# jacobkrantz/VLN-CE

Hardware: AMD Instinct MI355X
Metric: policy-steps/sec (fwd+bwd) (higher is better)
Workload: dtype f32

## Files before the change

vln-ce_amd/_lib.py:

```python
import ctypes as C
import os
import threading

import torch

_HERE = os.path.dirname(os.path.abspath(__file__))
LIB_PATH = os.environ.get("VLNCE_HIP_LIB") or os.path.join(_HERE, "libvlnce_hip.so")

_P = C.c_void_p
_I = C.c_int
_F = C.c_float
_L = C.c_long


def _buffer_format(explicit, *bufs):
    tags = {getattr(b, "_vlnce_fmt", None) for b in bufs if b is not None} - {None}
    if explicit:
        tags.add(int(explicit))
    if len(tags) > 1:
        raise RuntimeError(f"weight buffers / w_format disagree on the plane format: {sorted(tags)}")
    return tags.pop() if tags else 1


class ConvDesc(C.Structure):
# ... 102 lines not shown
    "vlnce_adaptive_avgpool_bwd": (_I, [_P, _P, _I, _I, _I, _I, _I, _I, _P]),
    "vlnce_rnn_seq_supported": (_I, [_I, _I]),
    "vlnce_rnn_seq_fwd": (_I, [_I, _I, _P, _P, _P, _P, _P, _P, _P, _P, _I, _I, _I, _P]),
    "vlnce_rnn_seq_bwd": (_I, [_I, _I, _P, _P, _P, _P, _P, _P, _P, _P, _P, _I, _I, _I, _P]),
    "vlnce_option_count": (_I, []),
    "vlnce_option_index": (_I, [C.c_char_p]),
    "vlnce_linear_rows_supported": (_I, [_I, _I, _I]),
    "vlnce_linear_rows_fwd": (_I, [_P, _I, _P, _I, _P, _I, _P, _I, _I, _I, _I, _P]),
    "vlnce_linear_rows_bwd": (_I, [_P, _I, _P, _I, _P, _I, _P, _I, _I, _P, _P, _P, _I, _I, _I, _P]),
    "vlnce_rnn_seq_fwd2": (_I, [_I, _I, _P, _P, _P, _P, _P, _P, _L, _L, _P, _P, _P, _I, _I, _I, _P]),
    "vlnce_rnn_seq_bwd2": (_I, [_I, _I, _P, _P, _P, _P, _P, _P, _L, _L, _P, _P, _P, _P, _I, _I, _I, _P]),
    "vlnce_rnn_seq_wgrad": (_I, [_I, _I, _I, _P, _P, _P, _P, _I, _I, _P, _P, _P, _P, _P, _P, _I, _I, _I, _P]),
    "vlnce_group_norm_small": (_I, [_P, _I, _I, _I, _I, _P, _P, _F, _P, _I, _P, _P]),
    "vlnce_gru_rollout_supported": (_I, [_I, _I]),
    "vlnce_gru_rollout_workspace_bytes": (C.c_long, [_I, _I]),
    "vlnce_gru_rollout_fwd": (_I, [_P, _P, _P, _P, _P, _P, _P, _P, _P, _P, _I, _I, _I, _P]),
    "vlnce_gru_rollout_bwd": (_I, [_P, _P, _P, _P, _P, _P, _P, _P, _P, _P, _P, _I, _I, _I, _P]),
    "vlnce_rnn_step_supported": (_I, [_I, _I, _I]),
    "vlnce_rnn_step_fwd": (_I, [_I, _P, _P, _P, _P, _P, _P, _P, _P, _P, _P, _I, _I, _P]),
    "vlnce_rnn_step_bwd": (_I, [_I, _P, _P, _P, _P, _P, _P, _P, _P, _P, _P, _P, _P, _P, _I, _I, _P]),
    "vlnce_select_rows": (_I, [_P, _P, _P, _P, _I, _I, _P]),
    "vlnce_act_bwd": (_I, [_P, _P, _P, _L, _I, _P]),
}


def exported_symbols():
    return sorted(_SIGNATURES)


def load_cdll(path=LIB_PATH):
    if not os.path.exists(path):
        raise RuntimeError(
            f"{path} not found: build it with `python __graft_entry__.py` (hipcc, gfx950). "
            "The VLN-CE policy path has no CPU fallback."
        )
    dll = C.CDLL(path)
    for name, (res, args) in _SIGNATURES.items():
        fn = getattr(dll, name)
        fn.restype = res
        fn.argtypes = args
    return dll


class _CallState(threading.local):
    dev = None
    restore = None


_CALL = _CallState()


def _ptr(t):
    if t is None:
        return None
    if not t.is_cuda:
        raise RuntimeError("libvlnce_hip: tensor is not on a GPU (no CPU fallback)")
    idx = t.device.index
    if _CALL.dev is None:
        _CALL.dev = idx
    elif _CALL.dev != idx:
        first, _CALL.dev = _CALL.dev, None
        raise RuntimeError(f"libvlnce_hip: tensors of one call live on cuda:{first} and "
                           f"cuda:{idx}")
    return t.data_ptr()


def _stream():
    dev, _CALL.dev = _CALL.dev, None
    if dev is None:
        return torch.cuda.current_stream().cuda_stream
    cur = torch.cuda.current_device()
    if dev != cur:
        _CALL.restore = cur
        torch.cuda.set_device(dev)
    return torch.cuda.current_stream(dev).cuda_stream


def _leave_device():
    if _CALL.restore is not None:
        cur, _CALL.restore = _CALL.restore, None
        torch.cuda.set_device(cur)


class HipLib:

    name = "hip"

    ABI = 143

    def __init__(self, path=LIB_PATH):
        self.dll = load_cdll(path)
        have = int(self.dll.vlnce_version())
        if have != self.ABI:
            raise RuntimeError(f"{path} has ABI {have}, this package binds ABI {self.ABI}: "
                               "rebuild it (python __graft_entry__.py)")

        self._conv_math = None
        self._tls = threading.local()
        self._options_from_env()

    OPTION_NAMES = ("conv_math", "p3", "p3_tile", "s3", "u3", "u3_waves", "x3_tile", "igemm_tile",
                    "igemm_nobuf", "igemm_no_splitk", "wgrad_tile", "rollout_one_xcd", "m3")

    def _options_from_env(self):
        for name in self.OPTION_NAMES:
            v = os.environ.get("VLNCE_" + name.upper())
            if v is None:
                continue
            if name == "conv_math":
                v = {"f32": 0, "0": 0, "bf16": 1, "1": 1, "f16": 2, "2": 2}.get(v.strip().lower(), v)
            elif name in ("igemm_nobuf", "igemm_no_splitk"):
                v = 0 if v in ("", "0") else 1
            try:
                v = int(v)
            except ValueError:
                import warnings
                warnings.warn(f"VLNCE_{name.upper()}={v!r} is not an integer: ignored "
                              f"(the option keeps its default)")
                continue
            self.set_option(name, v)

    def set_option(self, name, value):
        self._check(self.dll.vlnce_set_option(name.encode(), int(value)), "vlnce_set_option")
        if name == "conv_math":
            self._conv_math = int(value)

    def plane_format(self, options=None):
        v = None
        if options:
            v = options.get("conv_math")
        if v is None:
            sc = getattr(self._tls, "scoped", None)
            if sc:
                v = sc.get("conv_math")
        if v is None or v < 0:
            v = self._conv_math
            if v is None:
                v = self._conv_math = self.get_option("conv_math")
        return 2 if v == 2 else 1

    def get_option(self, name):
        v = _I(0)
        self._check(self.dll.vlnce_get_option(name.encode(), C.byref(v)), "vlnce_get_option")
        return v.value

    def option_default(self, name):
        v = _I(0)
        self._check(self.dll.vlnce_option_default(name.encode(), C.byref(v)), "vlnce_option_default")
        return v.value

    PER_LAUNCH = ("conv_math", "p3", "p3_tile", "s3", "u3", "u3_waves", "x3_tile", "m3")

    def _launch_options(self, overrides):
        if not overrides:
            return None
        arr = (C.c_int * int(self.dll.vlnce_option_count()))(*([-1] * int(self.dll.vlnce_option_count())))
        for name, v in overrides.items():
            i = int(self.dll.vlnce_option_index(name.encode()))
            if i < 0:
                raise RuntimeError(f"unknown dispatch option {name!r}")
            arr[i] = int(v)
        return arr

    def options(self, **kw):
        lib = self
        unknown = [k for k in kw if k not in self.OPTION_NAMES]
        if unknown:
            raise RuntimeError(f"unknown dispatch option(s) {unknown}")

        class _Scope:
            def __enter__(self_inner):
                self_inner.prev = getattr(lib._tls, "scoped", None)
                scoped = dict(self_inner.prev or {})
                scoped.update({k: v for k, v in kw.items() if k in lib.PER_LAUNCH})
                lib._tls.scoped = scoped or None
                self_inner.old = {k: lib.get_option(k) for k in kw if k not in lib.PER_LAUNCH}
                for k in self_inner.old:
                    lib.set_option(k, kw[k])
                return lib

            def __exit__(self_inner, *exc):
                lib._tls.scoped = self_inner.prev
                for k, v in self_inner.old.items():
                    lib.set_option(k, v)
                return False
# ... 338 lines not shown

    def gn_bwd_workspace_floats(self, Nimg, HW, Cc, groups):
        return int(self.dll.vlnce_gn_bwd_workspace_floats(Nimg, HW, Cc, groups))

    def gn_bwd(self, dy, y, x, mean, rstd, gamma, Nimg, HW, Cc, groups, relu, dx, dres, dgamma,
               dbeta, workspace, pow2=None):
        self._check(self.dll.vlnce_gn_bwd(_ptr(dy), _ptr(y), _ptr(x), _ptr(mean), _ptr(rstd),
                                          _ptr(gamma), Nimg, HW, Cc, groups, int(relu), _ptr(dx),
                                          _ptr(dres), _ptr(dgamma), _ptr(dbeta), _ptr(workspace),
                                          _ptr(pow2), pow2.size(1) if pow2 is not None else 0,
                                          _stream()), "vlnce_gn_bwd")

    def maxpool3x3s2_argmax(self, x, y, argmax, N, H, W, Cc, Ho, Wo):
        self._check(self.dll.vlnce_maxpool3x3s2_argmax(_ptr(x), _ptr(y), _ptr(argmax), N, H, W, Cc,
                                                       Ho, Wo, _stream()),
                    "vlnce_maxpool3x3s2_argmax")

    def maxpool3x3s2_bwd(self, dy, argmax, dx, N, H, W, Cc, Ho, Wo):
        self._check(self.dll.vlnce_maxpool3x3s2_bwd(_ptr(dy), _ptr(argmax), _ptr(dx), N, H, W, Cc,
                                                    Ho, Wo, _stream()), "vlnce_maxpool3x3s2_bwd")

    def adaptive_avgpool_bwd(self, dy, dx, N, H, W, Cc, OH, OW):
        self._check(self.dll.vlnce_adaptive_avgpool_bwd(_ptr(dy), _ptr(dx), N, H, W, Cc, OH, OW,
                                                        _stream()), "vlnce_adaptive_avgpool_bwd")

    @staticmethod
    def _parr(ts, n):
        if ts is None:
            return None
        arr = (C.c_void_p * 2)()
        for i in range(n):
            arr[i] = _ptr(ts[i])
        return arr

    def rnn_seq_supported(self, kind, H):
        return bool(self.dll.vlnce_rnn_seq_supported(kind, H))

    def rnn_seq_fwd(self, kind, dirs, gi, w_hh, b_hh, lengths, out, h_final, gates_save, aux_save,
                    B, Lm, H):
        pa = self._parr
        self._check(self.dll.vlnce_rnn_seq_fwd(
            kind, dirs, pa(gi, dirs), pa(w_hh, dirs), pa(b_hh, dirs), _ptr(lengths), pa(out, dirs),
            pa(h_final, dirs), pa(gates_save, dirs), pa(aux_save, dirs), B, Lm, H, _stream()),
            "vlnce_rnn_seq_fwd")

    def rnn_seq_bwd(self, kind, dirs, w_hh_t, lengths, out, gates_save, aux_save, dout, dh_final,
                    dgi, dgh, B, Lm, H):
        pa = self._parr
        self._check(self.dll.vlnce_rnn_seq_bwd(
            kind, dirs, pa(w_hh_t, dirs), _ptr(lengths), pa(out, dirs), pa(gates_save, dirs),
            pa(aux_save, dirs), pa(dout, dirs), pa(dh_final, dirs), pa(dgi, dirs), pa(dgh, dirs),
            B, Lm, H, _stream()), "vlnce_rnn_seq_bwd")

    def linear_rows_supported(self, M, N, K):
        return bool(self.dll.vlnce_linear_rows_supported(M, N, K))

    def linear_rows_fwd(self, x, ldx, w, ldw, bias, act, y, ldy, M, N, K):
        self._check(self.dll.vlnce_linear_rows_fwd(_ptr(x), ldx, _ptr(w), ldw, _ptr(bias), act, _ptr(y),
                                                   ldy, M, N, K, _stream()), "vlnce_linear_rows_fwd")

    def linear_rows_bwd(self, x, ldx, w, ldw, dy, lddy, y, ldy, act, dx, dw, db, M, N, K):
        self._check(self.dll.vlnce_linear_rows_bwd(_ptr(x), ldx, _ptr(w), ldw, _ptr(dy), lddy, _ptr(y),
                                                   ldy, act, _ptr(dx), _ptr(dw), _ptr(db), M, N, K,
                                                   _stream()), "vlnce_linear_rows_bwd")

    def rnn_seq_fwd2(self, kind, dirs, gi, w_hh, b_hh, lengths, out_tm, seq, seq_st, seq_sb, h_final,
                     gates_save, aux_save, B, Lm, H):
        pa = self._parr
        self._check(self.dll.vlnce_rnn_seq_fwd2(
            kind, dirs, pa(gi, dirs), pa(w_hh, dirs), pa(b_hh, dirs), _ptr(lengths), pa(out_tm, dirs),
            _ptr(seq), seq_st, seq_sb, pa(h_final, dirs), pa(gates_save, dirs), pa(aux_save, dirs),
            B, Lm, H, _stream()), "vlnce_rnn_seq_fwd2")

    def rnn_seq_bwd2(self, kind, dirs, w_hh, lengths, out_tm, gates_save, aux_save, dseq, dseq_st,
                     dseq_sb, dout_ws, dh_final, dgi, dgh, B, Lm, H):
        pa = self._parr
        self._check(self.dll.vlnce_rnn_seq_bwd2(
            kind, dirs, pa(w_hh, dirs), _ptr(lengths), pa(out_tm, dirs), pa(gates_save, dirs),
            pa(aux_save, dirs), _ptr(dseq), dseq_st, dseq_sb, _ptr(dout_ws), pa(dh_final, dirs),
            pa(dgi, dirs), pa(dgh, dirs), B, Lm, H, _stream()), "vlnce_rnn_seq_bwd2")

    def rnn_seq_wgrad(self, kind, dirs, dgi, dgh, out_tm, x_tm, ldx, E, w_ih, dw_ih, dw_hh, db_ih,
                      db_hh, dx_tm, B, Lm, H, first_dir=0):
        pa = self._parr
        self._check(self.dll.vlnce_rnn_seq_wgrad(
            kind, dirs, first_dir, pa(dgi, dirs), pa(dgh, dirs), pa(out_tm, dirs), _ptr(x_tm), ldx, E,
            pa(w_ih, dirs), pa(dw_ih, dirs), pa(dw_hh, dirs), pa(db_ih, dirs), pa(db_hh, dirs),
            _ptr(dx_tm), B, Lm, H, _stream()), "vlnce_rnn_seq_wgrad")

    def group_norm_small(self, x, N, HW, Cc, groups, gamma, beta, eps, residual, act, y):
        self._check(self.dll.vlnce_group_norm_small(
            _ptr(x), N, HW, Cc, groups, _ptr(gamma), _ptr(beta), eps, _ptr(residual), act, _ptr(y),
            _stream()), "vlnce_group_norm_small")

    def gru_rollout_supported(self, N, H):
        if os.environ.get("VLNCE_GRU_ROLLOUT", "1") == "0":
            return False
        return bool(self.dll.vlnce_gru_rollout_supported(N, H))

    def gru_rollout_workspace_bytes(self, N, H):
        return int(self.dll.vlnce_gru_rollout_workspace_bytes(N, H))

    def gru_rollout_fwd(self, gi, h0, mask, w_hh, b_hh, hp, out, gates, aux, workspace, T, N, H):
        self._check(self.dll.vlnce_gru_rollout_fwd(
            _ptr(gi), _ptr(h0), _ptr(mask), _ptr(w_hh), _ptr(b_hh), _ptr(hp), _ptr(out),
            _ptr(gates), _ptr(aux), _ptr(workspace), T, N, H, _stream()), "vlnce_gru_rollout_fwd")

    def gru_rollout_bwd(self, dout, dh_final, gates, aux, hp, mask, w_hh_t, dgi, dgh, dh0,
                        workspace, T, N, H):
        self._check(self.dll.vlnce_gru_rollout_bwd(
            _ptr(dout), _ptr(dh_final), _ptr(gates), _ptr(aux), _ptr(hp), _ptr(mask),
            _ptr(w_hh_t), _ptr(dgi), _ptr(dgh), _ptr(dh0), _ptr(workspace), T, N, H, _stream()),
            "vlnce_gru_rollout_bwd")

    def rnn_step_supported(self, N, H, lstm):
        if os.environ.get("VLNCE_RNN_STEP_FUSED", "1") == "0":
            return False
        return bool(self.dll.vlnce_rnn_step_supported(N, H, int(lstm)))

    def rnn_step_fwd(self, lstm, gi, h_prev, c_prev, mask, w_hh, b_hh, hp_out, h_out, aux_out,
                     gates_out, N, H):
        self._check(self.dll.vlnce_rnn_step_fwd(
            int(lstm), _ptr(gi), _ptr(h_prev), _ptr(c_prev), _ptr(mask), _ptr(w_hh), _ptr(b_hh),
            _ptr(hp_out), _ptr(h_out), _ptr(aux_out), _ptr(gates_out), N, H, _stream()),
            "vlnce_rnn_step_fwd")

    def rnn_step_bwd(self, lstm, dout, carry, dc, gates, aux, hp, c_prev, mask, w_hh_t, dgi, dgh,
                     acc0, dc_prev, N, H):
        self._check(self.dll.vlnce_rnn_step_bwd(
            int(lstm), _ptr(dout), _ptr(carry), _ptr(dc), _ptr(gates), _ptr(aux), _ptr(hp),
            _ptr(c_prev), _ptr(mask), _ptr(w_hh_t), _ptr(dgi), _ptr(dgh), _ptr(acc0),
            _ptr(dc_prev), N, H, _stream()), "vlnce_rnn_step_bwd")

    def select_rows(self, mask, a, b, out, B, H):
        self._check(self.dll.vlnce_select_rows(_ptr(mask), _ptr(a), _ptr(b), _ptr(out), B, H,
                                               _stream()), "vlnce_select_rows")

    def embedding_bwd(self, tokens, grad_rows, grad_weight, padding_idx):
        self._check(self.dll.vlnce_embedding_bwd(_ptr(tokens), _ptr(grad_rows), _ptr(grad_weight),
                                                 tokens.numel(), grad_weight.size(1),
                                                 -1 if padding_idx is None else int(padding_idx),
                                                 grad_weight.size(0), _stream()),
                    "vlnce_embedding_bwd")

    def act_bwd(self, dy, y, dz, n, act):
        self._check(self.dll.vlnce_act_bwd(_ptr(dy), _ptr(y), _ptr(dz), n, act, _stream()),
                    "vlnce_act_bwd")


_LIB = None


def get_lib():
    global _LIB
    if _LIB is None:
        _LIB = HipLib()
    return _LIB
```

vln-ce_amd/csrc/api.cpp:

```cpp
#include <stdarg.h>
#include <stdio.h>
#include <string.h>

#include <atomic>

#include "common_opts.h"

static thread_local char g_err[512] = "";

void vlnce_set_error(const char* fmt, ...) {
  va_list ap;
  va_start(ap, fmt);
  vsnprintf(g_err, sizeof(g_err), fmt, ap);
  va_end(ap);
}

extern "C" const char* vlnce_last_error(void) { return g_err; }
extern "C" int vlnce_version(void) { return 143; }

namespace {
struct OptDef {
  const char* name;
  int def;
};
const OptDef kOpts[VLNCE_OPT_COUNT] = {
    {"conv_math", 2},   {"p3", 2},          {"p3_tile", 0},         {"s3", 1},
    {"u3", 1},          {"u3_waves", 8},    {"x3_tile", 0},         {"igemm_tile", 0},
    {"igemm_nobuf", 0}, {"igemm_no_splitk", 0}, {"wgrad_tile", 64}, {"rollout_one_xcd", 0},
    {"m3", 1},
};
std::atomic<int> g_opt[VLNCE_OPT_COUNT] = {
    {2}, {2}, {0}, {1}, {1}, {8}, {0}, {0}, {0}, {0}, {64}, {0}, {1},
};
int opt_index(const char* name) {
  if (name)
    for (int i = 0; i < VLNCE_OPT_COUNT; ++i)
      if (strcmp(name, kOpts[i].name) == 0) return i;
  return -1;
}
}

namespace {
thread_local const int* t_call_opts = nullptr;
}
VlnceOptScope::VlnceOptScope(const int* per_call) : prev(t_call_opts) { t_call_opts = per_call; }
VlnceOptScope::~VlnceOptScope() { t_call_opts = prev; }

int vlnce_opt(int id) {
  if (t_call_opts && t_call_opts[id] >= 0) return t_call_opts[id];
  return g_opt[id].load(std::memory_order_relaxed);
}

extern "C" int vlnce_option_count(void) { return VLNCE_OPT_COUNT; }

extern "C" int vlnce_option_index(const char* name) { return opt_index(name); }

extern "C" int vlnce_set_option(const char* name, int value) {
  const int i = opt_index(name);
  if (i < 0) {
    vlnce_set_error("vlnce_set_option: unknown option '%s'", name ? name : "(null)");
    return 1;
  }
  g_opt[i].store(value, std::memory_order_relaxed);
  return 0;
}

extern "C" int vlnce_get_option(const char* name, int* value) {
  const int i = opt_index(name);
  if (i < 0 || !value) {
    vlnce_set_error("vlnce_get_option: unknown option '%s'", name ? name : "(null)");
    return 1;
  }
  *value = g_opt[i].load(std::memory_order_relaxed);
  return 0;
}

extern "C" int vlnce_option_default(const char* name, int* value) {
  const int i = opt_index(name);
  if (i < 0 || !value) {
    vlnce_set_error("vlnce_option_default: unknown option '%s'", name ? name : "(null)");
    return 1;
  }
  *value = kOpts[i].def;
  return 0;
}
```

vln-ce_amd/csrc/common_opts.h:

```cpp
#pragma once
#include "../../include/vlnce_hip.h"

void vlnce_set_error(const char* fmt, ...);

enum {
  VLNCE_OPT_CONV_MATH,
  VLNCE_OPT_P3,
  VLNCE_OPT_P3_TILE,
  VLNCE_OPT_S3,
  VLNCE_OPT_U3,
  VLNCE_OPT_U3_WAVES,
  VLNCE_OPT_X3_TILE,
  VLNCE_OPT_IGEMM_TILE,
  VLNCE_OPT_IGEMM_NOBUF,
  VLNCE_OPT_IGEMM_NO_SPLITK,
  VLNCE_OPT_WGRAD_TILE,
  VLNCE_OPT_ROLLOUT_ONE_XCD,
  VLNCE_OPT_M3,
  VLNCE_OPT_COUNT
};
int vlnce_opt(int id);

struct VlnceOptScope {
  explicit VlnceOptScope(const int* per_call);
  ~VlnceOptScope();
  const int* prev;
};
```

vln-ce_amd/csrc/rnn_seq.hip:

```cpp
#include "common.h"

namespace {

struct RnnSeqParams {
  const float* gi[2];
  const float* w_hh[2];
  const float* b_hh[2];
  float* out[2];
  float* h_final[2];
  float* gates[2];
  float* aux[2];
  const float* dout[2];
  const float* dh_final[2];
  float* dgi[2];
  float* dgh[2];
  const int* lengths;
  int B, L;
  float* seq[2];
  long seq_st, seq_sb;
  int self_zero;
  int w_plain;
};

__global__ __launch_bounds__(256) void dseq_to_time_major_kernel(const float* __restrict__ dseq, long st,
// ... 448 lines not shown
            const float dz = dht * (hp - ng);
            const float dnp = dn * (1.f - ng * ng);
            dpre[0] = dnp * hn * rg * (1.f - rg);
            dpre[1] = dz * zg * (1.f - zg);
            dpre[2] = dnp;
            dgh_n = dnp * rg;
            keep_z[nt][r] = dht * zg;
          }
          float* dgi = p.dgi[d] + base * GH;
#pragma unroll
          for (int gt = 0; gt < G; ++gt) dgi[gt * H + u] = dpre[gt];
          if (KIND == 1) {
            float* dgh = p.dgh[d] + base * GH;
            dgh[u] = dpre[0];
            dgh[H + u] = dpre[1];
            dgh[2 * H + u] = dgh_n;
          }
        }
#pragma unroll
        for (int gt = 0; gt < G; ++gt) {
          unsigned short dw[3];
          split_scalar((KIND == 1 && gt == 2) ? dgh_n : dpre[gt], dw);
#pragma unroll
          for (int q = 0; q < 3; ++q) dg_pl[q][row_i][gt * H + u] = dw[q];
        }
      }
    }
#ifdef RNN_SEQ_DBG_TIME
    const long long d_t1 = clock64();
#endif
    __syncthreads();
#ifdef RNN_SEQ_DBG_TIME
    const long long d_t2 = clock64();
#endif
    f32x4 acc[NTW];
#pragma unroll
    for (int nt = 0; nt < NTW; ++nt) acc[nt] = f32x4{0.f, 0.f, 0.f, 0.f};
#pragma unroll
    for (int ks = 0; ks < KS; ++ks) {
      bf16x8 a[3];
#pragma unroll
      for (int q = 0; q < 3; ++q)
        a[q] = *reinterpret_cast<const bf16x8*>(&dg_pl[q][l15][32 * ks + 8 * quad]);
      Planes3 wl;
      const bool from_lds = KL > 0 && ks >= KS - KL;
      if (from_lds) {
#pragma unroll
        for (int q = 0; q < 3; ++q) wl.p[q] = w_lds[KL > 0 ? ks - (KS - KL) : 0][q][tid];
      }
#pragma unroll
      for (int q = 0; q < 6; ++q)
#pragma unroll
        for (int nt = 0; nt < NTW; ++nt) {
          const bf16x8 wb = (from_lds && nt == 0) ? wl.p[X3_PB[q]] : wt[nt][ks].p[X3_PB[q]];
          acc[nt] = __builtin_amdgcn_mfma_f32_16x16x32_bf16(a[X3_PA[q]], wb, acc[nt], 0, 0, 0);
        }
    }
#pragma unroll
    for (int r = 0; r < 4; ++r) {
      const bool active = s < len[r];
      if (active)
#pragma unroll
        for (int nt = 0; nt < NTW; ++nt) dh[nt][r] = acc[nt][r] + keep_z[nt][r];
    }
#ifdef RNN_SEQ_DBG_TIME
    const long long d_t3 = clock64();
#endif
    __syncthreads();
#ifdef RNN_SEQ_DBG_TIME
    const long long d_t4 = clock64();
    d_a += d_t1 - d_t0;
    d_b1 += d_t2 - d_t1;
    d_m += d_t3 - d_t2;
    d_b2 += d_t4 - d_t3;
#endif
  }
#ifdef RNN_SEQ_DBG_TIME
  if (blockIdx.x == 0 && blockIdx.y == 0 && (tid == 0 || tid == 64 * (NW - 1)))
    printf("rnn_seq_bwd wave %d: %d steps; per step: gates+LDS write %lld, barrier %lld, reads+MFMA %lld, "
           "barrier %lld cycles\n", wave, Lt, d_a / Lt, d_b1 / Lt, d_m / Lt, d_b2 / Lt);
#endif
}

template <int KIND>
int launch_fwd(const RnnSeqParams& p, int H, int dirs, hipStream_t s) {
  dim3 grid(ceil_div(p.B, 16), dirs);
  if (H == 64)
    hipLaunchKernelGGL((rnn_seq_fwd_kernel<KIND, 64, 4>), grid, dim3(256), 0, s, p);
  else if (H == 128)
    hipLaunchKernelGGL((rnn_seq_fwd_kernel<KIND, 128, 8>), grid, dim3(512), 0, s, p);
  else
    return 1;
  return 0;
}
template <int KIND>
int launch_bwd(const RnnSeqParams& p, int H, int dirs, hipStream_t s) {
  dim3 grid(ceil_div(p.B, 16), dirs);
  if (H == 64)
    hipLaunchKernelGGL((rnn_seq_bwd_kernel<KIND, 64, 4>), grid, dim3(256), 0, s, p);
  else if (H == 128)
    hipLaunchKernelGGL((rnn_seq_bwd_kernel<KIND, 128, 8>), grid, dim3(512), 0, s, p);
  else
    return 1;
  return 0;
}

}

extern "C" int vlnce_rnn_seq_supported(int kind, int H) {
  return (kind == 0 || kind == 1) && (H == 64 || H == 128);
}

extern "C" int vlnce_rnn_seq_fwd(int kind, int dirs, const float* const* gi,
                                 const float* const* w_hh, const float* const* b_hh,
                                 const int* lengths, float* const* out, float* const* h_final,
                                 float* const* gates_save, float* const* aux_save, int B, int L,
                                 int H, vlnce_stream_t stream) {
  VLNCE_CHECK_ARG(gi && w_hh && b_hh && lengths && out && h_final, "rnn_seq_fwd: null argument");
  VLNCE_CHECK_ARG(dirs == 1 || dirs == 2, "rnn_seq_fwd: dirs must be 1 or 2");
  VLNCE_CHECK_ARG(vlnce_rnn_seq_supported(kind, H), "rnn_seq_fwd: unsupported kind/H (%d,%d)", kind, H);
  VLNCE_CHECK_ARG(B > 0 && L > 0, "rnn_seq_fwd: bad shape");
  RnnSeqParams p{};
  for (int d = 0; d < dirs; ++d) {
    p.gi[d] = gi[d];
    p.w_hh[d] = w_hh[d];
    p.b_hh[d] = b_hh[d];
    p.out[d] = out[d];
    p.h_final[d] = h_final[d];
    p.gates[d] = gates_save ? gates_save[d] : nullptr;
    p.aux[d] = aux_save ? aux_save[d] : nullptr;
    VLNCE_CHECK_ARG((p.gates[d] == nullptr) == (p.aux[d] == nullptr),
                    "rnn_seq_fwd: gates_save and aux_save come together");
  }
  p.lengths = lengths;
  p.B = B;
  p.L = L;
  hipStream_t s = reinterpret_cast<hipStream_t>(stream);
  const int rc = kind == 0 ? launch_fwd<0>(p, H, dirs, s) : launch_fwd<1>(p, H, dirs, s);
  VLNCE_CHECK_ARG(rc == 0, "rnn_seq_fwd: no kernel for H=%d", H);
  VLNCE_CHECK_LAUNCH("rnn_seq_fwd");
  return 0;
}

extern "C" int vlnce_rnn_seq_bwd(int kind, int dirs, const float* const* w_hh_t,
                                 const int* lengths, const float* const* out,
                                 const float* const* gates_save, const float* const* aux_save,
                                 const float* const* dout, const float* const* dh_final,
                                 float* const* dgi, float* const* dgh, int B, int L, int H,
                                 vlnce_stream_t stream) {
  VLNCE_CHECK_ARG(w_hh_t && lengths && out && gates_save && aux_save && dgi,
                  "rnn_seq_bwd: null argument");
  VLNCE_CHECK_ARG(dirs == 1 || dirs == 2, "rnn_seq_bwd: dirs must be 1 or 2");
  VLNCE_CHECK_ARG(vlnce_rnn_seq_supported(kind, H), "rnn_seq_bwd: unsupported kind/H (%d,%d)", kind, H);
  VLNCE_CHECK_ARG(kind == 0 || dgh, "rnn_seq_bwd: GRU needs dgh");
  RnnSeqParams p{};
  for (int d = 0; d < dirs; ++d) {
    p.w_hh[d] = w_hh_t[d];
    p.out[d] = const_cast<float*>(out[d]);
    p.gates[d] = const_cast<float*>(gates_save[d]);
    p.aux[d] = const_cast<float*>(aux_save[d]);
    p.dout[d] = dout ? dout[d] : nullptr;
    p.dh_final[d] = dh_final ? dh_final[d] : nullptr;
    p.dgi[d] = dgi[d];
    p.dgh[d] = dgh ? dgh[d] : nullptr;
  }
  p.lengths = lengths;
// ... 22 lines not shown
  for (int d = 0; d < dirs; ++d) {
    p.gi[d] = gi[d];
    p.w_hh[d] = w_hh[d];
    p.b_hh[d] = b_hh[d];
    p.out[d] = out_tm[d];
    p.seq[d] = seq ? seq + (long)d * H : nullptr;
    p.h_final[d] = h_final[d];
    p.gates[d] = gates_save ? gates_save[d] : nullptr;
    p.aux[d] = aux_save ? aux_save[d] : nullptr;
    VLNCE_CHECK_ARG((p.gates[d] == nullptr) == (p.aux[d] == nullptr),
                    "rnn_seq_fwd2: gates_save and aux_save come together");
  }
  p.seq_st = seq_st;
  p.seq_sb = seq_sb;
  p.self_zero = 1;
  p.lengths = lengths;
  p.B = B;
  p.L = L;
  hipStream_t s = reinterpret_cast<hipStream_t>(stream);
  const int rc = kind == 0 ? launch_fwd<0>(p, H, dirs, s) : launch_fwd<1>(p, H, dirs, s);
  VLNCE_CHECK_ARG(rc == 0, "rnn_seq_fwd2: no kernel for H=%d", H);
  VLNCE_CHECK_LAUNCH("rnn_seq_fwd2");
  return 0;
}

extern "C" int vlnce_rnn_seq_bwd2(int kind, int dirs, const float* const* w_hh, const int* lengths,
                                  const float* const* out_tm, const float* const* gates_save,
                                  const float* const* aux_save, const float* dseq, long dseq_st,
                                  long dseq_sb, float* dout_ws, const float* const* dh_final,
                                  float* const* dgi, float* const* dgh, int B, int L, int H,
                                  vlnce_stream_t stream) {
  VLNCE_CHECK_ARG(w_hh && lengths && out_tm && gates_save && aux_save && dgi,
                  "rnn_seq_bwd2: null argument");
  VLNCE_CHECK_ARG(dirs == 1 || dirs == 2, "rnn_seq_bwd2: dirs must be 1 or 2");
  VLNCE_CHECK_ARG(vlnce_rnn_seq_supported(kind, H), "rnn_seq_bwd2: unsupported kind/H (%d,%d)", kind, H);
  VLNCE_CHECK_ARG(kind == 0 || dgh, "rnn_seq_bwd2: GRU needs dgh");
  VLNCE_CHECK_ARG(!dseq || (dseq_st > 0 && dseq_sb > 0), "rnn_seq_bwd2: dseq needs its strides");
  VLNCE_CHECK_ARG(!dseq || dout_ws, "rnn_seq_bwd2: dseq needs the dirs*L*B*H workspace");
  hipStream_t s = reinterpret_cast<hipStream_t>(stream);
  if (dseq) {
    const long n4 = (long)dirs * L * B * (H / 4);
    const int grid = (int)((n4 + 255) / 256 > 2048 ? 2048 : (n4 + 255) / 256);
    hipLaunchKernelGGL(dseq_to_time_major_kernel, dim3(grid), dim3(256), 0, s, dseq, dseq_st, dseq_sb,
                       dout_ws, dirs, L, B, H);
    VLNCE_CHECK_LAUNCH("rnn_seq_bwd2 (output gradient to time-major)");
  }
  RnnSeqParams p{};
  for (int d = 0; d < dirs; ++d) {
    p.w_hh[d] = w_hh[d];
    p.out[d] = const_cast<float*>(out_tm[d]);
    p.gates[d] = const_cast<float*>(gates_save[d]);
    p.aux[d] = const_cast<float*>(aux_save[d]);
    p.dout[d] = dseq ? dout_ws + (long)d * L * B * H : nullptr;
    p.dh_final[d] = dh_final ? dh_final[d] : nullptr;
    p.dgi[d] = dgi[d];
    p.dgh[d] = dgh ? dgh[d] : nullptr;
  }
  p.self_zero = 1;
  p.w_plain = 1;
  p.lengths = lengths;
  p.B = B;
  p.L = L;
  const int rc = kind == 0 ? launch_bwd<0>(p, H, dirs, s) : launch_bwd<1>(p, H, dirs, s);
  VLNCE_CHECK_ARG(rc == 0, "rnn_seq_bwd2: no kernel for H=%d", H);
  VLNCE_CHECK_LAUNCH("rnn_seq_bwd2");
  return 0;
}

extern "C" int vlnce_rnn_seq_wgrad(int kind, int dirs, int first_dir, const float* const* dgi,
                                   const float* const* dgh, const float* const* out_tm,
                                   const float* x_tm, int ldx, int E, const float* const* w_ih,
                                   float* const* dw_ih, float* const* dw_hh, float* const* db_ih,
                                   float* const* db_hh, float* dx_tm, int B, int L, int H,
                                   vlnce_stream_t stream) {
  VLNCE_CHECK_ARG(dgi && out_tm && x_tm && dw_ih && dw_hh && db_ih && db_hh,
                  "rnn_seq_wgrad: null argument");
  VLNCE_CHECK_ARG(dirs == 1 || dirs == 2, "rnn_seq_wgrad: dirs must be 1 or 2");
  VLNCE_CHECK_ARG((first_dir == 0 || first_dir == 1) && first_dir + dirs <= 2,
                  "rnn_seq_wgrad: first_dir + dirs must stay within the two directions");
  VLNCE_CHECK_ARG(kind == 0 || dgh, "rnn_seq_wgrad: GRU needs dgh");
  VLNCE_CHECK_ARG(!dx_tm || w_ih, "rnn_seq_wgrad: dx_tm needs w_ih");
  const int GH = (kind == 0 ? 4 : 3) * H;
  const long rows = (long)L * B;
  VLNCE_CHECK_ARG(B > 0 && L > 0 && E > 0 && ldx >= E && rows < 0x7fffffffL, "rnn_seq_wgrad: bad shape");
  hipStream_t s = reinterpret_cast<hipStream_t>(stream);
  for (int d = 0; d < dirs; ++d) {
    const float* dGh = kind == 1 ? dgh[d] : dgi[d];
    if (L > 1) {
      const bool reverse = first_dir + d == 1;
      const float* dG_s = reverse ? dGh : dGh + (long)B * GH;
      const float* h_s = reverse ? out_tm[d] + (long)B * H : out_tm[d];
      int rc = vlnce_gemm(dG_s, GH, 1, h_s, H, 1, dw_hh[d], H, GH, H, (int)((long)(L - 1) * B), nullptr, stream);
      if (rc != 0) return rc;
    } else {
      vlnce_zero(dw_hh[d], GH, H, H, s);
    }
    int rc = vlnce_colsum(dGh, GH, (int)rows, GH, db_hh[d], 0, stream);
    if (rc != 0) return rc;
    rc = vlnce_gemm(dgi[d], GH, 1, x_tm, ldx, 1, dw_ih[d], E, GH, E, (int)rows, nullptr, stream);
    if (rc != 0) return rc;
    if (db_ih[d] != db_hh[d]) {
      rc = vlnce_colsum(dgi[d], GH, (int)rows, GH, db_ih[d], 0, stream);
      if (rc != 0) return rc;
    }
    if (dx_tm) {
      vlnce_epilogue e{};
      e.accumulate = d > 0;
      rc = vlnce_gemm(dgi[d], GH, 0, w_ih[d], E, 1, dx_tm, E, (int)rows, E, GH, &e, stream);
      if (rc != 0) return rc;
    }
  }
  return 0;
}
```

vln-ce_amd/ops.py:

```python
import os

import torch
import torch.nn.functional as F
from torch.autograd import Function

from . import _lib

ACT_NONE, ACT_RELU, ACT_SIGMOID, ACT_TANH = 0, 1, 2, 3


def L():
    return _lib.get_lib()


def _f32c(t):
    if t.dtype != torch.float32:
        t = t.float()
    return t if t.is_contiguous() else t.contiguous()


def _rows2d(t):
    if t.dim() != 2 or t.stride(1) != 1 or (t.size(0) > 1 and t.stride(0) < t.size(1)):
        t = t.reshape(-1, t.size(-1)).contiguous()
    ld = t.stride(0) if t.size(0) > 1 else t.size(1)
# ... 940 lines not shown
            torch.mul(acc, mf[t], out=carry)
        dw = torch.empty_like(w_hh)
        lib.gemm(dgh.view(T * N, GH), GH, 1, hp.view(T * N, H), H, 1, dw, H, GH, H, T * N)
        db = torch.empty((GH,), device=dev, dtype=torch.float32)
        lib.colsum(dgh.view(T * N, GH), GH, T * N, GH, db, 0)
        dc0 = dc if lstm else None
        return None, dgi.view(T * N, GH), carry, dc0, None, dw, db


class RNNLayerFn(Function):

    @staticmethod
    def forward(ctx, kind, save, lengths, dirs, B, Lm, x_tm, *params):
        x_tm, ldx = _rows2d(_f32c(x_tm) if x_tm.dtype != torch.float32 else x_tm)
        E = x_tm.size(1)
        w_ih = [_f32c(params[4 * d]) for d in range(dirs)]
        b_ih = [params[4 * d + 1] for d in range(dirs)]
        w_hh = [_f32c(params[4 * d + 2]) for d in range(dirs)]
        b_hh = [_f32c(params[4 * d + 3]) for d in range(dirs)]
        GH, H = w_hh[0].shape
        dev = x_tm.device
        lib = L()
        rows = Lm * B
        gis = []
        for d in range(dirs):
            gi = torch.empty((rows, GH), device=dev, dtype=torch.float32)
            if not _planes_gemm(x_tm, ldx, w_ih[d], gi, b_ih[d]):
                lib.gemm(x_tm, ldx, 0, w_ih[d], E, 0, gi, GH, rows, GH, E, shift=b_ih[d])
            gis.append(gi.view(Lm, B, GH))

        def new(*shape):
            return torch.empty(shape, device=dev, dtype=torch.float32)

        out_tm = [new(Lm, B, H) for _ in range(dirs)]
        seq = new(B, Lm, dirs * H)
        hfin = [new(B, H) for _ in range(dirs)]
        gates = aux = None
        if save:
            gates = [new(Lm, B, GH) for _ in range(dirs)]
            aux = [new(Lm, B, H) for _ in range(dirs)]
        lib.rnn_seq_fwd2(kind, dirs, gis, w_hh, b_hh, lengths, out_tm, seq, dirs * H, Lm * dirs * H,
                         hfin, gates, aux, B, Lm, H)
        ctx.cfg = (kind, dirs, Lm, B, H, GH, E, ldx)
        ctx.set_materialize_grads(False)
        if save:
            ctx.save_for_backward(lengths, x_tm, *w_ih, *w_hh, *out_tm, *gates, *aux)
        return (seq, *hfin)

    @staticmethod
    def backward(ctx, dseq, *dhf):
        kind, dirs, Lm, B, H, GH, E, ldx = ctx.cfg
        sv = ctx.saved_tensors
        lengths, x_tm = sv[0], sv[1]
        w_ih, w_hh = sv[2:2 + dirs], sv[2 + dirs:2 + 2 * dirs]
        out_tm = sv[2 + 2 * dirs:2 + 3 * dirs]
        gates = sv[2 + 3 * dirs:2 + 4 * dirs]
        aux = sv[2 + 4 * dirs:2 + 5 * dirs]
        dev = x_tm.device
        st = sb = 0
        if dseq is not None:
            if (dseq.dtype != torch.float32 or dseq.stride(2) != 1 or dseq.stride(0) <= 0
                    or dseq.stride(1) <= 0):
                dseq = _f32c(dseq)
            sb, st = dseq.stride(0), dseq.stride(1)
        dhf = [(_f32c(g) if g is not None else None) for g in dhf[:dirs]]

        def new(*shape):
            return torch.empty(shape, device=dev, dtype=torch.float32)

        dgi = [new(Lm, B, GH) for _ in range(dirs)]
        dgh = [new(Lm, B, GH) for _ in range(dirs)] if kind == 1 else None
        lib = L()
        ws = new(dirs, Lm, B, H) if dseq is not None else None
        lib.rnn_seq_bwd2(kind, dirs, list(w_hh), lengths, list(out_tm), list(gates), list(aux), dseq,
                         st, sb, ws, dhf, dgi, dgh, B, Lm, H)
        dw_ih = [new(GH, E) for _ in range(dirs)]
        dw_hh = [new(GH, H) for _ in range(dirs)]
        db_ih = [new(GH) for _ in range(dirs)]
        db_hh = [new(GH) for _ in range(dirs)]
        need_dx = ctx.needs_input_grad[6]
        dx = new(Lm * B, E) if need_dx else None
        from .streams import BranchStreams

        if (dirs == 2 and Lm * B >= 2048 and BranchStreams.enabled(dev)
                and os.environ.get("VLNCE_RNN_WGRAD_STREAMS", "1") != "0"):
            cur = torch.cuda.current_stream(dev)
            side = BranchStreams()._stream(1, dev)
            if side is cur:
                side = BranchStreams()._stream(2, dev)
            dx1 = new(Lm * B, E) if need_dx else None
            fork = torch.cuda.Event()
            fork.record(cur)
            side.wait_event(fork)
            with torch.cuda.stream(side):
                lib.rnn_seq_wgrad(kind, 1, dgi[1:], dgh[1:] if dgh else None, list(out_tm[1:]), x_tm, ldx, E,
                                  list(w_ih[1:]), dw_ih[1:], dw_hh[1:], db_ih[1:], db_hh[1:], dx1, B, Lm,
                                  H, first_dir=1)
                done = torch.cuda.Event()
                done.record(side)
            lib.rnn_seq_wgrad(kind, 1, dgi[:1], dgh[:1] if dgh else None, list(out_tm[:1]), x_tm, ldx, E,
                              list(w_ih[:1]), dw_ih[:1], dw_hh[:1], db_ih[:1], db_hh[:1], dx, B, Lm, H)
            cur.wait_event(done)
            if need_dx:
                dx.add_(dx1)
        else:
            lib.rnn_seq_wgrad(kind, dirs, dgi, dgh, list(out_tm), x_tm, ldx, E, list(w_ih), dw_ih, dw_hh,
                              db_ih, db_hh, dx, B, Lm, H)
        res = [None, None, None, None, None, None, dx]
        for d in range(dirs):
            res += [dw_ih[d], db_ih[d], dw_hh[d], db_hh[d]]
        return tuple(res)


def rnn_layer(kind, lengths_i32, x_tm, B, Lm, per_direction, need_grad):
    flat = [t for quad in per_direction for t in quad]
    res = RNNLayerFn.apply(kind, bool(need_grad), lengths_i32, len(per_direction), B, Lm, x_tm, *flat)
    return res[0], list(res[1:])
```

Measured before the change: 8052.

## Fuse RNN weight-gradient GEMMs and bias colsums into one MFMA kernel

Adds a single kernel that computes dW_hh, dW_ih, db_hh and db_ih for both directions with 32x32 f32 MFMA tiles, a reduction over the rows split across 16 waves, and the time shift handled by index arithmetic. It replaces the per-direction GEMM and colsum launches and turns off the two-stream split for the wgrad, so the dx GEMM stays on one stream. The aim is fewer launches and reading the gate gradients once for both the weight and bias sums. The cost is that each block does a long serial walk over the rows with no split-K across blocks, which may under-use the GPU when the row count is large.

```diff
diff --git a/vln-ce_amd/_lib.py b/vln-ce_amd/_lib.py
--- a/vln-ce_amd/_lib.py
+++ b/vln-ce_amd/_lib.py
@@ -208,11 +208,15 @@
         torch.cuda.set_device(cur)
 
 
+def tail_fused():
+    return os.environ.get("VLNCE_TAIL_FUSED", "1") != "0"
+
+
 class HipLib:
 
     name = "hip"
 
-    ABI = 143
+    ABI = 144
 
     def __init__(self, path=LIB_PATH):
         self.dll = load_cdll(path)
@@ -226,7 +230,8 @@
         self._options_from_env()
 
     OPTION_NAMES = ("conv_math", "p3", "p3_tile", "s3", "u3", "u3_waves", "x3_tile", "igemm_tile",
-                    "igemm_nobuf", "igemm_no_splitk", "wgrad_tile", "rollout_one_xcd", "m3")
+                    "igemm_nobuf", "igemm_no_splitk", "wgrad_tile", "rollout_one_xcd", "m3",
+                    "rnn_wgrad_fused")
 
     def _options_from_env(self):
         for name in self.OPTION_NAMES:
@@ -731,6 +736,15 @@
 
     def rnn_seq_wgrad(self, kind, dirs, dgi, dgh, out_tm, x_tm, ldx, E, w_ih, dw_ih, dw_hh, db_ih,
                       db_hh, dx_tm, B, Lm, H, first_dir=0):
+        if not tail_fused():
+            with self.options(rnn_wgrad_fused=0):
+                return self._rnn_seq_wgrad(kind, dirs, first_dir, dgi, dgh, out_tm, x_tm, ldx, E, w_ih,
+                                           dw_ih, dw_hh, db_ih, db_hh, dx_tm, B, Lm, H)
+        self._rnn_seq_wgrad(kind, dirs, first_dir, dgi, dgh, out_tm, x_tm, ldx, E, w_ih, dw_ih, dw_hh,
+                            db_ih, db_hh, dx_tm, B, Lm, H)
+
+    def _rnn_seq_wgrad(self, kind, dirs, first_dir, dgi, dgh, out_tm, x_tm, ldx, E, w_ih, dw_ih, dw_hh,
+                       db_ih, db_hh, dx_tm, B, Lm, H):
         pa = self._parr
         self._check(self.dll.vlnce_rnn_seq_wgrad(
             kind, dirs, first_dir, pa(dgi, dirs), pa(dgh, dirs), pa(out_tm, dirs), _ptr(x_tm), ldx, E,
diff --git a/vln-ce_amd/csrc/api.cpp b/vln-ce_amd/csrc/api.cpp
--- a/vln-ce_amd/csrc/api.cpp
+++ b/vln-ce_amd/csrc/api.cpp
@@ -16,7 +16,7 @@
 }
 
 extern "C" const char* vlnce_last_error(void) { return g_err; }
-extern "C" int vlnce_version(void) { return 143; }
+extern "C" int vlnce_version(void) { return 144; }
 
 namespace {
 struct OptDef {
@@ -27,10 +27,10 @@
     {"conv_math", 2},   {"p3", 2},          {"p3_tile", 0},         {"s3", 1},
     {"u3", 1},          {"u3_waves", 8},    {"x3_tile", 0},         {"igemm_tile", 0},
     {"igemm_nobuf", 0}, {"igemm_no_splitk", 0}, {"wgrad_tile", 64}, {"rollout_one_xcd", 0},
-    {"m3", 1},
+    {"m3", 1},          {"rnn_wgrad_fused", 1},
 };
 std::atomic<int> g_opt[VLNCE_OPT_COUNT] = {
-    {2}, {2}, {0}, {1}, {1}, {8}, {0}, {0}, {0}, {0}, {64}, {0}, {1},
+    {2}, {2}, {0}, {1}, {1}, {8}, {0}, {0}, {0}, {0}, {64}, {0}, {1}, {1},
 };
 int opt_index(const char* name) {
   if (name)
diff --git a/vln-ce_amd/csrc/common_opts.h b/vln-ce_amd/csrc/common_opts.h
--- a/vln-ce_amd/csrc/common_opts.h
+++ b/vln-ce_amd/csrc/common_opts.h
@@ -17,6 +17,7 @@
   VLNCE_OPT_WGRAD_TILE,
   VLNCE_OPT_ROLLOUT_ONE_XCD,
   VLNCE_OPT_M3,
+  VLNCE_OPT_RNN_WGRAD_FUSED,
   VLNCE_OPT_COUNT
 };
 int vlnce_opt(int id);
diff --git a/vln-ce_amd/csrc/rnn_seq.hip b/vln-ce_amd/csrc/rnn_seq.hip
--- a/vln-ce_amd/csrc/rnn_seq.hip
+++ b/vln-ce_amd/csrc/rnn_seq.hip
@@ -554,6 +554,97 @@
 #endif
 }
 
+struct RnnWgradParams {
+  const float* dgi[2];
+  const float* dgh[2];
+  const float* out[2];
+  float* dw_ih[2];
+  float* dw_hh[2];
+  float* db_ih[2];
+  float* db_hh[2];
+  const float* x;
+  int ldx, E;
+  int reverse[2];
+  int rows, B, H, GH;
+  int nq;
+  int nth, nt;
+};
+constexpr int WGRAD_WAVES = 16;
+constexpr int WGRAD_U = 8;
+
+__global__ __launch_bounds__(WGRAD_WAVES * 64) void rnn_seq_wgrad_kernel(RnnWgradParams p) {
+  __shared__ float red[WGRAD_WAVES / 2][16][64];
+  __shared__ float bred[WGRAD_WAVES][64];
+  const int tid = threadIdx.x, lane = tid & 63, wave = tid >> 6;
+  const int slot = blockIdx.x >> 3;
+  const int q = (slot / p.nt) * 8 + (blockIdx.x & 7);
+  if (q >= p.nq) return;
+  const int n = slot % p.nt;
+  const int qpd = p.GH / 32;
+  const int d = q / qpd, i0 = (q - d * qpd) * 32;
+  const bool hh = n < p.nth;
+  const int j0 = (hh ? n : n - p.nth) * 32;
+  const int l31 = lane & 31, kh = lane >> 5;
+
+  const float* __restrict__ a_src = (hh ? p.dgh[d] : p.dgi[d]) + i0 + l31;
+  const float* __restrict__ b_src = hh ? p.out[d] + j0 + l31 : p.x + j0 + l31;
+  const int ldb = hh ? p.H : p.ldx;
+  const int shift = hh ? (p.reverse[d] ? p.B : -p.B) : 0;
+  const bool col_ok = hh || j0 + l31 < p.E;
+  const int rows = p.rows;
+
+  f32x16 acc;
+#pragma unroll
+  for (int v = 0; v < 16; ++v) acc[v] = 0.f;
+  float bs = 0.f;
+  for (int r0 = wave * (2 * WGRAD_U); r0 < rows; r0 += WGRAD_WAVES * 2 * WGRAD_U) {
+    float a[WGRAD_U], b[WGRAD_U];
+#pragma unroll
+    for (int u = 0; u < WGRAD_U; ++u) {
+      const int r = r0 + 2 * u + kh;
+      const int rb = r + shift;
+      a[u] = r < rows ? a_src[(long)r * p.GH] : 0.f;
+      b[u] = (col_ok && r < rows && rb >= 0 && rb < rows) ? b_src[(long)rb * ldb] : 0.f;
+    }
+#pragma unroll
+    for (int u = 0; u < WGRAD_U; ++u) {
+      bs += a[u];
+      acc = __builtin_amdgcn_mfma_f32_32x32x2f32(a[u], b[u], acc, 0, 0, 0);
+    }
+  }
+
+  if (wave >= WGRAD_WAVES / 2) {
+#pragma unroll
+    for (int v = 0; v < 16; ++v) red[wave - WGRAD_WAVES / 2][v][lane] = acc[v];
+  }
+  bred[wave][lane] = bs;
+  __syncthreads();
+  if (wave < WGRAD_WAVES / 2) {
+#pragma unroll
+    for (int v = 0; v < 16; ++v) red[wave][v][lane] += acc[v];
+  }
+  __syncthreads();
+  {
+    const int v = wave;
+    float s = 0.f;
+#pragma unroll
+    for (int w = 0; w < WGRAD_WAVES / 2; ++w) s += red[w][v][lane];
+    const int row = i0 + (v & 3) + 8 * (v >> 2) + 4 * kh;
+    const int col = j0 + l31;
+    if (hh)
+      p.dw_hh[d][(long)row * p.H + col] = s;
+    else if (col < p.E)
+      p.dw_ih[d][(long)row * p.E + col] = s;
+  }
+  float* db = n == 0 ? p.db_hh[d] : n == p.nth ? p.db_ih[d] : nullptr;
+  if (db && tid < 32) {
+    float s = 0.f;
+#pragma unroll
+    for (int w = 0; w < WGRAD_WAVES; ++w) s += bred[w][tid] + bred[w][tid + 32];
+    db[i0 + tid] = s;
+  }
+}
+
 template <int KIND>
 int launch_fwd(const RnnSeqParams& p, int H, int dirs, hipStream_t s) {
   dim3 grid(ceil_div(p.B, 16), dirs);
@@ -742,26 +833,60 @@
   VLNCE_CHECK_ARG(!dx_tm || w_ih, "rnn_seq_wgrad: dx_tm needs w_ih");
   const int GH = (kind == 0 ? 4 : 3) * H;
   const long rows = (long)L * B;
-  VLNCE_CHECK_ARG(B > 0 && L > 0 && E > 0 && ldx >= E && rows < 0x7fffffffL, "rnn_seq_wgrad: bad shape");
+  VLNCE_CHECK_ARG(B > 0 && L > 0 && E > 0 && H > 0 && ldx >= E && rows < 0x7fffffffL - 2L * B - 512,
+                  "rnn_seq_wgrad: bad shape");
   hipStream_t s = reinterpret_cast<hipStream_t>(stream);
+  const bool fused = H % 32 == 0 && vlnce_opt(VLNCE_OPT_RNN_WGRAD_FUSED) != 0;
+  if (fused) {
+    RnnWgradParams p{};
+    for (int d = 0; d < dirs; ++d) {
+      VLNCE_CHECK_ARG(dgi[d] && out_tm[d] && dw_ih[d] && dw_hh[d] && db_ih[d] && db_hh[d] &&
+                          (kind == 0 || dgh[d]),
+                      "rnn_seq_wgrad: null argument");
+      p.dgi[d] = dgi[d];
+      p.dgh[d] = kind == 1 ? dgh[d] : dgi[d];
+      p.out[d] = out_tm[d];
+      p.dw_ih[d] = dw_ih[d];
+      p.dw_hh[d] = dw_hh[d];
+      p.db_hh[d] = db_hh[d];
+      p.db_ih[d] = db_ih[d] != db_hh[d] ? db_ih[d] : nullptr;
+      p.reverse[d] = first_dir + d == 1;
+    }
+    p.x = x_tm;
+    p.ldx = ldx;
+    p.E = E;
+    p.rows = (int)rows;
+    p.B = B;
+    p.H = H;
+    p.GH = GH;
+    p.nq = dirs * (GH / 32);
+    p.nth = H / 32;
+    p.nt = p.nth + ceil_div(E, 32);
+    const int grid = ceil_div(p.nq, 8) * 8 * p.nt;
+    hipLaunchKernelGGL(rnn_seq_wgrad_kernel, dim3(grid), dim3(WGRAD_WAVES * 64), 0, s, p);
+    VLNCE_CHECK_LAUNCH("rnn_seq_wgrad");
+  }
   for (int d = 0; d < dirs; ++d) {
-    const float* dGh = kind == 1 ? dgh[d] : dgi[d];
-    if (L > 1) {
-      const bool reverse = first_dir + d == 1;
-      const float* dG_s = reverse ? dGh : dGh + (long)B * GH;
-      const float* h_s = reverse ? out_tm[d] + (long)B * H : out_tm[d];
-      int rc = vlnce_gemm(dG_s, GH, 1, h_s, H, 1, dw_hh[d], H, GH, H, (int)((long)(L - 1) * B), nullptr, stream);
+    int rc = 0;
+    if (!fused) {
+      const float* dGh = kind == 1 ? dgh[d] : dgi[d];
+      if (L > 1) {
+        const bool reverse = first_dir + d == 1;
+        const float* dG_s = reverse ? dGh : dGh + (long)B * GH;
+        const float* h_s = reverse ? out_tm[d] + (long)B * H : out_tm[d];
+        rc = vlnce_gemm(dG_s, GH, 1, h_s, H, 1, dw_hh[d], H, GH, H, (int)((long)(L - 1) * B), nullptr, stream);
+        if (rc != 0) return rc;
+      } else {
+        vlnce_zero(dw_hh[d], GH, H, H, s);
+      }
+      rc = vlnce_colsum(dGh, GH, (int)rows, GH, db_hh[d], 0, stream);
       if (rc != 0) return rc;
-    } else {
-      vlnce_zero(dw_hh[d], GH, H, H, s);
-    }
-    int rc = vlnce_colsum(dGh, GH, (int)rows, GH, db_hh[d], 0, stream);
-    if (rc != 0) return rc;
-    rc = vlnce_gemm(dgi[d], GH, 1, x_tm, ldx, 1, dw_ih[d], E, GH, E, (int)rows, nullptr, stream);
-    if (rc != 0) return rc;
-    if (db_ih[d] != db_hh[d]) {
-      rc = vlnce_colsum(dgi[d], GH, (int)rows, GH, db_ih[d], 0, stream);
+      rc = vlnce_gemm(dgi[d], GH, 1, x_tm, ldx, 1, dw_ih[d], E, GH, E, (int)rows, nullptr, stream);
       if (rc != 0) return rc;
+      if (db_ih[d] != db_hh[d]) {
+        rc = vlnce_colsum(dgi[d], GH, (int)rows, GH, db_ih[d], 0, stream);
+        if (rc != 0) return rc;
+      }
     }
     if (dx_tm) {
       vlnce_epilogue e{};
diff --git a/vln-ce_amd/ops.py b/vln-ce_amd/ops.py
--- a/vln-ce_amd/ops.py
+++ b/vln-ce_amd/ops.py
@@ -1046,7 +1046,7 @@
         dx = new(Lm * B, E) if need_dx else None
         from .streams import BranchStreams
 
-        if (dirs == 2 and Lm * B >= 2048 and BranchStreams.enabled(dev)
+        if (dirs == 2 and Lm * B >= 2048 and BranchStreams.enabled(dev) and not _lib.tail_fused()
                 and os.environ.get("VLNCE_RNN_WGRAD_STREAMS", "1") != "0"):
             cur = torch.cuda.current_stream(dev)
             side = BranchStreams()._stream(1, dev)
```

Result: faster. 8134 (median of 6 runs) (+1.0%).
